# Shimly-2/DRL-on-robot-arm

Measured on AMD Instinct MI355X. Metric: env-steps/sec at N parallel envs (rl_reach_env), higher is better.
Workload: dtype f64

## Files before the change

drl-on-robot-arm_amd/csrc/armenv_env.h:

```cpp
#pragma once
#include "../../include/armenv.h"
#include "armenv_kin.h"
#include "armenv_actor.h"

using namespace armenv;


template <typename T> struct EnvCold {
  T q_init[NJ];
  T p_init[3];
  T trig_init[2 * NJ];
  T lim[2 * NJ + 1];
  double goal_lo[3], goal_hi[3];
  double push_rest_z, push_place_min, push_place_max, push_place_z;
  uint64_t seed, env_id0;
  int32_t push_model;
  int32_t fall_on;
  int32_t fall_land;
  T fall_c;
  T fall_keep;
  T place_z;
  T tool_radius, tool_below, erp_dt, split, fric_dv, dt;
};

// ... 266 lines not shown
    P.episode[i] = ep + 1u;
    if (goal_in) {
      g[0] = goal_in[3 * i]; g[1] = goal_in[3 * i + 1]; g[2] = goal_in[3 * i + 2];
    } else {
      sample_goal(P, i, ep, g);
    }
    static_for<0, NJ>([&](auto JI) { constexpr int j = JI; P.q[(int64_t)j * P.n + i] = P.cold->q_init[j]; });
    static_for<0, 2 * NJ>([&](auto JI) { constexpr int j = JI; P.trig[(int64_t)j * P.n + i] = P.cold->trig_init[j]; });
    static_for<0, 3>([&](auto KI) { constexpr int k = KI; P.goal[(int64_t)k * P.n + i] = g[k]; });
    P.step[i] = 0;
    P.ep_return[i] = T(0);
    if (obs) store_obs6<T>(obs, i, P.cold->p_init, g);
  }

  static AE_DEV double summary_distance(const EnvParams<T> &P, int64_t i) {
    T q[NJ], cq[NJ], sq[NJ];
    static_for<0, NJ>([&](auto JI) { constexpr int j = JI; q[j] = P.q[(int64_t)j * P.n + i]; });
    sincos_all<T>(q, cq, sq);
    FKState<T> S;
    fk<C, T>(P.chain, cq, sq, S);
    const T x = S.p[0] - (T)P.goal[0 * P.n + i], y = S.p[1] - (T)P.goal[1 * P.n + i], z = S.p[2] - (T)P.goal[2 * P.n + i];
    return (double)M::sqrt(M::fma(x, x, M::fma(y, y, z * z)));
  }

  T q[NJ];
  T cq[NJ], sq[NJ];
  FKState<T> S;
  AE_DEV void make_frame(const EnvParams<T> &P) { fk<C, T>(P.chain, cq, sq, S); }
  float g[3];
  int32_t step;
  T ep_ret;
  uint32_t n_done = 0, n_succ = 0, n_bad = 0, n_upd = 0;
  uint32_t n_lim = 0, n_low = 0, n_cap = 0, n_cond = 0;
  T minpiv = T(1e30);

  AE_DEV void load(const EnvParams<T> &P, int64_t i) {
    const int64_t n = P.n;
    static_for<0, NJ>([&](auto JI) { constexpr int j = JI; q[j] = P.q[(int64_t)j * n + i]; });
    static_for<0, 3>([&](auto KI) { constexpr int k = KI; g[k] = P.goal[(int64_t)k * n + i]; });
    step = P.step[i];
    ep_ret = P.ep_return[i];
    static_for<0, NJ>([&](auto JI) { constexpr int j = JI; cq[j] = P.trig[(int64_t)j * n + i]; sq[j] = P.trig[(int64_t)(NJ + j) * n + i]; });
  }
  AE_DEV void derive_trig() { sincos_all<T>(q, cq, sq); }

  AE_DEV void store(const EnvParams<T> &P, int64_t i) {
    const int64_t n = P.n;
    static_for<0, NJ>([&](auto JI) { constexpr int j = JI; P.q[(int64_t)j * n + i] = q[j]; });
    static_for<0, NJ>([&](auto JI) { constexpr int j = JI; P.trig[(int64_t)j * n + i] = cq[j]; P.trig[(int64_t)(NJ + j) * n + i] = sq[j]; });
    P.step[i] = step;
    P.ep_return[i] = ep_ret;
    flush_counts(P, i, n_done, n_succ, n_bad, n_upd, n_lim, n_low, n_cap, n_cond);
  }

  template <bool CARRY>
  AE_DEV void step_begin(const EnvParams<T> &P, const T (&a)[3], T (&tgt)[3]) {
    if constexpr (!CARRY) make_frame(P);
    ik_target<T, false>(S, a, P.dv, P.box_lo, P.box_hi, tgt);
    minpiv = T(1e30);
  }
  template <bool CARRY>
  AE_DEV void step_tail(const EnvParams<T> &P, int64_t i, const StepIO &io, int updates, bool lim_hit) {
    const int64_t n = P.n;
    n_upd += (uint32_t)updates;
    if constexpr (kFence) {
      n_lim += lim_hit ? 1u : 0u; n_low += (S.p[2] < P.fence_z) ? 1u : 0u; n_cap += (updates >= P.ik.max_iters) ? 1u : 0u;
      n_cond += (minpiv < P.ik.fence_pivot) ? 1u : 0u;
      if (io.updates) io.updates[i] = (uint8_t)(updates > 255 ? 255 : updates);
    }
    step += 1;
    const T dx = S.p[0] - (T)g[0], dy = S.p[1] - (T)g[1], dz = S.p[2] - (T)g[2];
    const T dist = M::sqrt(M::fma(dx, dx, M::fma(dy, dy, dz * dz)));
    const bool over = step > P.max_steps;
    const bool succ = !over & (dist < P.reach_dis);
    const bool done = over | succ;
    const T reward = succ ? T(0) : -dist * T(10);
    ep_ret += reward;
    if constexpr (kTipOf(kMode)) {
      if (io.diag) { io.diag[4 * i] = (double)S.p[0]; io.diag[4 * i + 1] = (double)S.p[1]; io.diag[4 * i + 2] = (double)S.p[2]; io.diag[4 * i + 3] = (double)reward; }
    }

    bool finite = true;
    {
      const T sum = ((q[0] + q[1]) + (q[2] + q[3])) + ((q[4] + q[5]) + q[6]);
      finite = M::finite(sum);
    }
    if (!finite) n_bad += 1;

    io.reward[i] = (float)reward;
    io.done[i] = done ? 1 : 0;
    io.success[i] = succ ? 1 : 0;
    if (__builtin_expect(io.terminal_obs != nullptr, 0)) store_obs6<T>(io.terminal_obs, i, S.p, g);

    const bool rederive = kTrigRederive > 0 && (step & (kTrigRederive - 1)) == 0;
    store_obs6<T>(io.obs, i, S.p, g);
    cur_obs[0] = (float)S.p[0]; cur_obs[1] = (float)S.p[1]; cur_obs[2] = (float)S.p[2];
    if (__builtin_expect(done | rederive, 0)) {
      if (done) {
        P.last_return[i] = ep_ret;
        P.last_len[i] = step;
        P.last_success[i] = succ ? 1 : 0;
        n_done += 1;
        if (succ) n_succ += 1;
      }
      if (done && P.auto_reset) {
        const uint32_t ep = P.episode[i];
        sample_goal(P, i, ep, g);
        P.episode[i] = ep + 1u;
        static_for<0, 3>([&](auto KI) { constexpr int k = KI; P.goal[(int64_t)k * n + i] = g[k]; });
        const EnvCold<T> &K = *P.cold;
        static_for<0, NJ>([&](auto JI) { constexpr int j = JI; q[j] = K.q_init[j]; });
        static_for<0, NJ>([&](auto JI) { constexpr int j = JI; cq[j] = K.trig_init[j]; sq[j] = K.trig_init[NJ + j]; });
        step = 0;
        ep_ret = T(0);
        store_obs6<T>(io.obs, i, K.p_init, g);
        cur_obs[0] = (float)K.p_init[0]; cur_obs[1] = (float)K.p_init[1]; cur_obs[2] = (float)K.p_init[2];
        if constexpr (CARRY) make_frame(P);
      } else if (rederive) {
        derive_trig();
        if constexpr (CARRY) make_frame(P);
      }
    }
  }
  template <bool CARRY = false, int PEEL = 0>
  AE_DEV int env_step(const EnvParams<T> &P, int64_t i, const T (&a)[3], const StepIO &io, ActionPrefetch *prefetched = nullptr,
                    float (*next_action)[3] = nullptr) {
    T tgt[3];
    step_begin<CARRY>(P, a, tgt);
    const int updates = ik_lockstep<C, T, kMode, PEEL>(P.chain, P.ik, q, tgt, S, cq, sq, minpiv);
    const bool lim_hit = ik_limits<C, T, kMode>(P.chain, P.ik, q, S, cq, sq);
    if (prefetched) prefetch_settle(*prefetched, *next_action);
    step_tail<CARRY>(P, i, io, updates, lim_hit);
    return updates;
  }

  float cur_obs[3];
  AE_DEV void refresh_obs(const EnvParams<T> &P) {
    FKState<T> F;
    fk<C, T>(P.chain, cq, sq, F);
    cur_obs[0] = (float)F.p[0]; cur_obs[1] = (float)F.p[1]; cur_obs[2] = (float)F.p[2];
  }
  AE_DEV void policy_obs(float (&s)[6]) const {
    s[0] = cur_obs[0]; s[1] = cur_obs[1]; s[2] = cur_obs[2]; s[3] = g[0]; s[4] = g[1]; s[5] = g[2];
  }
};

template <bool PICK, typename T>
AE_DEV void cube_sample(const EnvParams<T> &P, int64_t i, uint32_t episode, T (&cube)[3], T (&target)[3]) {
  const EnvCold<T> &K = *P.cold;
  double cx = 0, cy = 0, tx = 0, ty = 0, tz = K.push_place_z;
  constexpr uint32_t kBlocks = PICK ? 4u : 3u;
  for (uint32_t t = 0; t < 1000u; ++t) {
    double u0, u1, u2, u3, u4, u5;
    philox_pair(K.seed, K.env_id0 + (uint64_t)i, episode, kBlocks * t + 0u, u0, u1);
    philox_pair(K.seed, K.env_id0 + (uint64_t)i, episode, kBlocks * t + 1u, u2, u3);
    philox_pair(K.seed, K.env_id0 + (uint64_t)i, episode, kBlocks * t + 2u, u4, u5);
    cx = K.goal_lo[0] + (K.goal_hi[0] - K.goal_lo[0]) * u0;
    cy = K.goal_lo[1] + (K.goal_hi[1] - K.goal_lo[1]) * u1;
    tx = K.goal_lo[0] + (K.goal_hi[0] - K.goal_lo[0]) * u3;
    ty = K.goal_lo[1] + (K.goal_hi[1] - K.goal_lo[1]) * u4;
    const double dx = cx - tx, dy = cy - ty;
    double d;
    if constexpr (PICK) {
      tz = K.goal_lo[2] + (K.goal_hi[2] - K.goal_lo[2]) * u5;
      const double dz = K.push_place_z - tz;
      d = ::sqrt(::fma(dx, dx, ::fma(dy, dy, dz * dz)));
    } else {
// ... 182 lines not shown
      cube[2] = z < P.push_rest_z ? P.push_rest_z : z;
      return;
    }
    if (grip == T(0)) {
      const T h = P.push_cube_half;
      T g2 = T(0);
      static_for<0, 3>([&](auto KI) {
        constexpr int k = KI;
        const T lo = cube[k] - h, hi = cube[k] + h;
        const T c = tip[k] < lo ? lo : (tip[k] > hi ? hi : tip[k]);
        const T g = tip[k] - c;
        g2 = M::fma(g, g, g2);
      });
      if (M::sqrt(g2) - P.push_eef_radius < P.pick_trigger_dis) {
        const T hx = cube[0] - tip[0], hy = cube[1] - tip[1];
        const bool hold = tip[2] >= cube[2] && M::sqrt(M::fma(hx, hx, hy * hy)) <= P.pick_jaw_half;
        grip = hold ? T(2) : T(1);
        if (hold) {
          off[0] = hx; off[1] = hy; off[2] = cube[2] - tip[2];
          return;
        }
      }
    }
    contact(P, tip0, tip);
  }

  T p0[3];
  T q7s, c7s, s7s;
  template <bool CARRY>
  AE_DEV void step_begin(const EnvParams<T> &P, const T (&a)[3], T (&tgt)[3]) {
    if constexpr (PICK) { q7s = q[NJ - 1]; c7s = cq[NJ - 1]; s7s = sq[NJ - 1]; }
    if constexpr (!(CARRY && !PICK)) make_frame(P);
    p0[0] = S.p[0]; p0[1] = S.p[1]; p0[2] = S.p[2];
    ik_target<T, PICK>(S, a, P.dv, P.box_lo, P.box_hi, tgt);
    minpiv = T(1e30);
  }
  template <bool CARRY>
  AE_DEV void step_tail(const EnvParams<T> &P, int64_t i, const StepIO &io, int updates, bool lim_hit) {
    constexpr bool kCarry = CARRY && !PICK;
    n_upd += (uint32_t)updates;
    if constexpr (kFence) {
      n_lim += lim_hit ? 1u : 0u; n_low += (S.p[2] < P.fence_z) ? 1u : 0u; n_cap += (updates >= P.ik.max_iters) ? 1u : 0u;
      n_cond += (minpiv < P.ik.fence_pivot) ? 1u : 0u;
      if (io.updates) io.updates[i] = (uint8_t)(updates > 255 ? 255 : updates);
    }
    if constexpr (PICK) {
      q[NJ - 1] = q7s;
      cq[NJ - 1] = c7s; sq[NJ - 1] = s7s;
      const EnvCold<T> *Kp = P.cold;
      asm volatile("" : "+s"(Kp));
      if (Kp->fall_on && grip != T(2)) {
        if (step > 0) cube_fall(*Kp, 2 * step + 1);
        cube_fall(*Kp, 2 * step + 2);
      }
      grip_step(P, p0, S);
    } else {
      const EnvCold<T> *Kp = P.cold;
      asm volatile("" : "+s"(Kp));
      const EnvCold<T> &K = *Kp;
      if (K.push_model == 1) { cube_fall(K, step + 2); contact_dyn(P, K, S.p, step + 2); }
      else contact(P, p0, S.p);
    }
    step += 1;
    const T d_cur = dist_ct();
    T test = d_cur - d_last;
    if (M::fabs(test) < T(1e-5)) test = T(0.01);
    d_last = d_cur;
    const float fx = (float)cube[0] - (float)target[0], fy = (float)cube[1] - (float)target[1],
                fz = (float)cube[2] - (float)target[2];
    const float dt32 = sqrtf(fmaf(fx, fx, fmaf(fy, fy, fz * fz)));
    T reward;
    bool done;
    if (step > P.max_steps) { reward = (T)(-dt32 * 50.0f); done = true; }
    else if ((double)dt32 < (double)P.push_success_dis) { reward = T(100); done = true; }
    else { reward = -test * T(100); done = false; }
    const bool succ = d_cur < P.push_success_dis;
    ep_ret += reward;
    if constexpr (kTipOf(kMode)) {
      if (io.diag) { io.diag[4 * i] = (double)S.p[0]; io.diag[4 * i + 1] = (double)S.p[1]; io.diag[4 * i + 2] = (double)S.p[2]; io.diag[4 * i + 3] = (double)reward; }
    }

    bool finite = true;
    {
      const T sum = ((q[0] + q[1]) + (q[2] + q[3])) + ((q[4] + q[5]) + q[6]);
      finite = M::finite(sum);
    }
    if (!finite) n_bad += 1;

    io.reward[i] = (float)reward;
    io.done[i] = done ? 1 : 0;
    io.success[i] = succ ? 1 : 0;
    if (__builtin_expect(io.terminal_obs != nullptr, 0)) store_obs9<T>(io.terminal_obs, i, S.p, cube, target);
    const bool rederive = kTrigRederive > 0 && (step & (kTrigRederive - 1)) == 0;
    store_obs9<T>(io.obs, i, S.p, cube, target);
    cur_obs[0] = (float)S.p[0]; cur_obs[1] = (float)S.p[1]; cur_obs[2] = (float)S.p[2];
    if (__builtin_expect(done | rederive, 0)) {
      if (done) {
        P.last_return[i] = ep_ret;
        P.last_len[i] = step;
        P.last_success[i] = succ ? 1 : 0;
        n_done += 1;
        if (succ) n_succ += 1;
      }
      if (done && P.auto_reset) {
        const uint32_t ep = P.episode[i];
        cube_sample<PICK, T>(P, i, ep, cube, target);
        P.episode[i] = ep + 1u;
        d_last = dist_ct();
        if constexpr (PICK) { grip = T(0); off[0] = off[1] = off[2] = T(0); }
        else { vel[0] = vel[1] = T(0); }
        const EnvCold<T> &K = *P.cold;
        static_for<0, NJ>([&](auto JI) { constexpr int j = JI; q[j] = K.q_init[j]; });
        static_for<0, NJ>([&](auto JI) { constexpr int j = JI; cq[j] = K.trig_init[j]; sq[j] = K.trig_init[NJ + j]; });
        step = 0;
        ep_ret = T(0);
        store_obs9<T>(io.obs, i, K.p_init, cube, target);
        cur_obs[0] = (float)K.p_init[0]; cur_obs[1] = (float)K.p_init[1]; cur_obs[2] = (float)K.p_init[2];
        if constexpr (kCarry) make_frame(P);
      } else if (rederive) {
        derive_trig();
        if constexpr (kCarry) make_frame(P);
      }
    }
  }
  template <bool CARRY = false, int PEEL = 0>
  AE_DEV int env_step(const EnvParams<T> &P, int64_t i, const T (&a)[3], const StepIO &io, ActionPrefetch *prefetched = nullptr,
                    float (*next_action)[3] = nullptr) {
    T tgt[3];
    step_begin<CARRY>(P, a, tgt);
    const int updates = ik_lockstep<C, T, kMode, PEEL>(P.chain, P.ik, q, tgt, S, cq, sq, minpiv);
    const bool lim_hit = ik_limits<C, T, kMode>(P.chain, P.ik, q, S, cq, sq);
    if (prefetched) prefetch_settle(*prefetched, *next_action);
    step_tail<CARRY>(P, i, io, updates, lim_hit);
    return updates;
  }
};
template <class C, typename T, int MODE = 0> using PushLane = CubeLane<C, T, false, MODE>;
template <class C, typename T, int MODE = 0> using PickLane = CubeLane<C, T, true, MODE>;

template <class Lane, typename T>
__global__ __launch_bounds__(256) void env_reset_kernel(EnvParams<T> P, const uint8_t *mask, const float *goal_in, float *obs) {
  const int64_t i = (int64_t)blockIdx.x * blockDim.x + threadIdx.x;
  if (i >= P.n) return;
  if (mask && !mask[i]) return;
  Lane::reset_env(P, i, goal_in, obs);
}

template <class Lane, typename T, int WAVES = 1>
__global__ __launch_bounds__(256) __attribute__((amdgpu_waves_per_eu(WAVES, WAVES))) void env_step_kernel(EnvParams<T> P, StepIO io) {
  TL_STAMP(tl0);
#ifdef ARMENV_TIMELINE
  const unsigned tl_launch = __hip_atomic_load(&g_tl_launch, __ATOMIC_RELAXED, __HIP_MEMORY_SCOPE_AGENT);
#endif
  const int64_t i = lane_env(P);
  if (i < 0) return;
  if (i >= P.n) return;
  Lane L;
  L.load(P, i);
  T a[3];
  static_for<0, 3>([&](auto KI) { constexpr int k = KI; a[k] = (T)io.action[3 * i + k]; });
#ifdef ARMENV_TIMELINE
  asm volatile("s_waitcnt vmcnt(0)" ::: "memory");
#endif
  TL_STAMP(tl1);
  const int updates = L.template env_step<false, ARMENV_STEP_PEEL>(P, i, a, io);
  (void)updates;
  TL_STAMP(tl2);
// ... 343 lines not shown
```

drl-on-robot-arm_amd/csrc/armenv_kin.h:

```cpp
#pragma once
#include "armenv_math.h"
#include "chains_builtin.h"

namespace armenv {

constexpr bool kFenceOf(int mode) { return mode >= 1; }
constexpr bool kTipOf(int mode) { return mode == 2; }

template <typename T> struct ChainDev {
  T xyz[NJ][3];
  T R[NJ][9];
  T base_p[3];
  T base_R[9];
};

struct GenericChain {
  static constexpr bool kGeneric = true;
  static constexpr const char *kName = "generic";
};

template <typename T> struct IKParams {
  T tq[4];
  T lambda;
  T residual;
  T max_dtheta;
  int32_t max_iters;
  int32_t exit_mode;
  int32_t angle_f32;
  int32_t clamp_limits;
  int32_t pad0;
  T fence_pivot;
  T tip[3];
  const T *lim;
  T lim_min;
};

template <typename T> struct FKState {
  T W[9];
  T p[3];
  T z[NJ][3];
  T pj[NJ][3];
};

template <class C> struct FkKinds {
  int Wk[NJ + 1][9];
  int Ak[NJ][9];
  constexpr FkKinds() : Wk{}, Ak{} {
    for (int i = 0; i < 9; ++i) Wk[0][i] = (i % 4 == 0) ? 2 : 1;
    for (int j = 0; j < NJ; ++j) {
      for (int c = 0; c < 3; ++c) {
        const int k = C::perm[j][c], sg = C::sgn[j][c];
        for (int r = 0; r < 3; ++r) {
          const int w = Wk[j][3 * k + r];
          Ak[j][3 * c + r] = (sg > 0 || w < 2) ? w : (w == 2 ? 3 : 2);
        }
      }
      for (int r = 0; r < 3; ++r) {
        const bool z = Ak[j][r] == 1 && Ak[j][3 + r] == 1;
        Wk[j + 1][r] = z ? 1 : 0;
        Wk[j + 1][3 + r] = z ? 1 : 0;
        Wk[j + 1][6 + r] = Ak[j][6 + r];
      }
    }
  }
};
template <int KA, int KB, typename T>
AE_DEV T rot_term(T c, T a, T s, T b) {
  using M = Mth<T>;
  if constexpr (KA == 1 && KB == 1) return T(0);
  else if constexpr (KA == 1) return KB == 2 ? s : (KB == 3 ? -s : s * b);
  else if constexpr (KB == 1) return KA == 2 ? c : (KA == 3 ? -c : c * a);
  else if constexpr (KA >= 2) return (KA == 2 ? c : -c) + (KB == 2 ? s : (KB == 3 ? -s : s * b));
  else return M::fma(c, a, KB == 2 ? s : (KB == 3 ? -s : s * b));
}

template <class C, typename T>
AE_DEV void fk(const ChainDev<T> &ch, const T (&cq)[NJ], const T (&sq)[NJ], FKState<T> &S) {
  using M = Mth<T>;
  if constexpr (C::kGeneric) {
    static_for<0, 9>([&](auto I) { constexpr int i = I; S.W[3 * (i % 3) + (i / 3)] = ch.base_R[i]; });
    static_for<0, 3>([&](auto I) { constexpr int i = I; S.p[i] = ch.base_p[i]; });
  } else {
    static_for<0, 9>([&](auto I) { constexpr int i = I; S.W[i] = (i % 4 == 0) ? T(1) : T(0); });
    static_for<0, 3>([&](auto I) { constexpr int i = I; S.p[i] = T(0); });
  }
  static_for<0, NJ>([&](auto JI) {
    constexpr int j = JI;
    T A[9];
    if constexpr (C::kGeneric) {
      static_for<0, 3>([&](auto RI) {
        constexpr int r = RI;
        S.p[r] = M::fma(S.W[0 + r], ch.xyz[j][0], M::fma(S.W[3 + r], ch.xyz[j][1], M::fma(S.W[6 + r], ch.xyz[j][2], S.p[r])));
      });
      static_for<0, 3>([&](auto CI) {
        constexpr int c = CI;
        static_for<0, 3>([&](auto RI) {
          constexpr int r = RI;
          A[3 * c + r] = M::fma(S.W[0 + r], ch.R[j][0 + c], M::fma(S.W[3 + r], ch.R[j][3 + c], S.W[6 + r] * ch.R[j][6 + c]));
        });
      });
    } else {
      static_for<0, 3>([&](auto KI) {
        constexpr int k = KI;
        constexpr double t = C::xyz[j][k];
        if constexpr (t != 0.0) {
          static_for<0, 3>([&](auto RI) {
            constexpr int r = RI;
            constexpr int kw = FkKinds<C>().Wk[j][3 * k + r];
            if constexpr (kw == 0) S.p[r] = M::fma(S.W[3 * k + r], T(t), S.p[r]);
            else if constexpr (kw == 2) S.p[r] = S.p[r] + T(t);
            else if constexpr (kw == 3) S.p[r] = S.p[r] - T(t);
          });
        }
      });
      static_for<0, 3>([&](auto CI) {
        constexpr int c = CI;
        constexpr int k = C::perm[j][c];
        constexpr int s = C::sgn[j][c];
        static_for<0, 3>([&](auto RI) { constexpr int r = RI; A[3 * c + r] = (s > 0) ? S.W[3 * k + r] : -S.W[3 * k + r]; });
      });
    }
    const T sn = sq[j], cs = cq[j];
    static_for<0, 3>([&](auto RI) {
      constexpr int r = RI;
      if constexpr (C::kGeneric) {
        S.W[0 + r] = M::fma(cs, A[0 + r], sn * A[3 + r]);
        S.W[3 + r] = M::fma(cs, A[3 + r], -(sn * A[0 + r]));
      } else {
        constexpr int k0 = FkKinds<C>().Ak[j][0 + r], k3 = FkKinds<C>().Ak[j][3 + r];
        constexpr int k0n = k0 < 2 ? k0 : (k0 == 2 ? 3 : 2);
        S.W[0 + r] = rot_term<k0, k3, T>(cs, A[0 + r], sn, A[3 + r]);
        S.W[3 + r] = rot_term<k3, k0n, T>(cs, A[3 + r], sn, -A[0 + r]);
      }
      S.W[6 + r] = A[6 + r];
      S.z[j][r] = A[6 + r];
      S.pj[j][r] = S.p[r];
    });
  });
}

template <typename T>
AE_DEV void sincos_kernel(T r, T &s, T &c) {
  using M = Mth<T>;
  const T z = r * r;
  T ps = T(1.58969099521155010221e-10);
  ps = M::fma(ps, z, T(-2.50507602534068634195e-08));
  ps = M::fma(ps, z, T(2.75573137070700676789e-06));
  ps = M::fma(ps, z, T(-1.98412698298579493134e-04));
  ps = M::fma(ps, z, T(8.33333333332248946124e-03));
  ps = M::fma(ps, z, T(-1.66666666666666324348e-01));
  s = M::fma(r * z, ps, r);
  T pc = T(-1.13596475577881948265e-11);
  pc = M::fma(pc, z, T(2.08757232129817482790e-09));
  pc = M::fma(pc, z, T(-2.75573143513906633035e-07));
  pc = M::fma(pc, z, T(2.48015872894767294178e-05));
  pc = M::fma(pc, z, T(-1.38888888888741095749e-03));
  pc = M::fma(pc, z, T(4.16666666666666019037e-02));
  c = M::fma(z * z, pc, M::fma(T(-0.5), z, T(1)));
}

AE_DEV void sincos_joint(double x, double &s, double &c) {
  if (!(::fabs(x) < 1.0e5)) { ::sincos(x, &s, &c); return; }
  const double k = ::rint(x * 6.36619772367581382433e-01);
  double r = ::fma(-k, 1.57079632673412561417e+00, x);
  r = ::fma(-k, 6.07710050630396597660e-11, r);
  r = ::fma(-k, 2.02226624871116645580e-21, r);
  r = ::fma(-k, 8.47842766036889956997e-32, r);
  double sr, cr;
  sincos_kernel<double>(r, sr, cr);
  const int n = (int)k & 3;
  const double s1 = (n & 1) ? cr : sr, c1 = (n & 1) ? sr : cr;
  s = (n & 2) ? -s1 : s1;
  c = ((n + 1) & 2) ? -c1 : c1;
}
AE_DEV void sincos_joint(float x, float &s, float &c) { ::sincosf(x, &s, &c); }

template <typename T>
AE_DEV void sincos_all(const T (&q)[NJ], T (&cq)[NJ], T (&sq)[NJ]) {
  static_for<0, NJ>([&](auto JI) { constexpr int j = JI; sincos_joint(q[j], sq[j], cq[j]); });
}
template <>
AE_DEV void sincos_all<double>(const double (&q)[NJ], double (&cq)[NJ], double (&sq)[NJ]) {
  double k[NJ], r[NJ], z[NJ], ps[NJ], pc[NJ];
  static_for<0, NJ>([&](auto JI) { constexpr int j = JI; k[j] = ::rint(q[j] * 6.36619772367581382433e-01); });
  static_for<0, NJ>([&](auto JI) { constexpr int j = JI; r[j] = ::fma(-k[j], 1.57079632673412561417e+00, q[j]); });
  static_for<0, NJ>([&](auto JI) { constexpr int j = JI; r[j] = ::fma(-k[j], 6.07710050630396597660e-11, r[j]); });
  static_for<0, NJ>([&](auto JI) { constexpr int j = JI; r[j] = ::fma(-k[j], 2.02226624871116645580e-21, r[j]); });
  static_for<0, NJ>([&](auto JI) { constexpr int j = JI; r[j] = ::fma(-k[j], 8.47842766036889956997e-32, r[j]); z[j] = r[j] * r[j]; });
  static_for<0, NJ>([&](auto JI) { constexpr int j = JI; ps[j] = ::fma(1.58969099521155010221e-10, z[j], -2.50507602534068634195e-08); });
  static_for<0, NJ>([&](auto JI) { constexpr int j = JI; ps[j] = ::fma(ps[j], z[j], 2.75573137070700676789e-06); });
  static_for<0, NJ>([&](auto JI) { constexpr int j = JI; ps[j] = ::fma(ps[j], z[j], -1.98412698298579493134e-04); });
  static_for<0, NJ>([&](auto JI) { constexpr int j = JI; ps[j] = ::fma(ps[j], z[j], 8.33333333332248946124e-03); });
  static_for<0, NJ>([&](auto JI) { constexpr int j = JI; ps[j] = ::fma(ps[j], z[j], -1.66666666666666324348e-01); });
  static_for<0, NJ>([&](auto JI) { constexpr int j = JI; pc[j] = ::fma(-1.13596475577881948265e-11, z[j], 2.08757232129817482790e-09); });
  static_for<0, NJ>([&](auto JI) { constexpr int j = JI; pc[j] = ::fma(pc[j], z[j], -2.75573143513906633035e-07); });
  static_for<0, NJ>([&](auto JI) { constexpr int j = JI; pc[j] = ::fma(pc[j], z[j], 2.48015872894767294178e-05); });
  static_for<0, NJ>([&](auto JI) { constexpr int j = JI; pc[j] = ::fma(pc[j], z[j], -1.38888888888741095749e-03); });
  static_for<0, NJ>([&](auto JI) { constexpr int j = JI; pc[j] = ::fma(pc[j], z[j], 4.16666666666666019037e-02); });
  static_for<0, NJ>([&](auto JI) {
    constexpr int j = JI;
    const double sr = ::fma(r[j] * z[j], ps[j], r[j]);
    const double cr = ::fma(z[j] * z[j], pc[j], ::fma(-0.5, z[j], 1.0));
    const int n = (int)k[j] & 3;
    const double s1 = (n & 1) ? cr : sr, c1 = (n & 1) ? sr : cr;
    sq[j] = (n & 2) ? -s1 : s1;
    cq[j] = ((n + 1) & 2) ? -c1 : c1;
  });
}
template <>
AE_DEV void sincos_all<float>(const float (&q)[NJ], float (&cq)[NJ], float (&sq)[NJ]) {
  float k[NJ], r[NJ], z[NJ], ps[NJ], pc[NJ];
  static_for<0, NJ>([&](auto JI) { constexpr int j = JI; k[j] = ::rintf(q[j] * 0.636619772f); });
  static_for<0, NJ>([&](auto JI) { constexpr int j = JI; r[j] = ::fmaf(-k[j], 1.5703125f, q[j]); });
  static_for<0, NJ>([&](auto JI) { constexpr int j = JI; r[j] = ::fmaf(-k[j], 4.837512969970703125e-4f, r[j]); });
  static_for<0, NJ>([&](auto JI) { constexpr int j = JI; r[j] = ::fmaf(-k[j], 7.54978995489188216e-8f, r[j]); z[j] = r[j] * r[j]; });
  static_for<0, NJ>([&](auto JI) { constexpr int j = JI; ps[j] = ::fmaf(2.7183114939898219064e-6f, z[j], -1.98393348360966317347e-4f); });
  static_for<0, NJ>([&](auto JI) { constexpr int j = JI; ps[j] = ::fmaf(ps[j], z[j], 8.3333293858894631756e-3f); });
  static_for<0, NJ>([&](auto JI) { constexpr int j = JI; ps[j] = ::fmaf(ps[j], z[j], -1.66666666416265235595e-1f); });
  static_for<0, NJ>([&](auto JI) { constexpr int j = JI; pc[j] = ::fmaf(2.43904487962774090654e-5f, z[j], -1.38867637746099294692e-3f); });
  static_for<0, NJ>([&](auto JI) { constexpr int j = JI; pc[j] = ::fmaf(pc[j], z[j], 4.16666233237390631894e-2f); });
  static_for<0, NJ>([&](auto JI) { constexpr int j = JI; pc[j] = ::fmaf(pc[j], z[j], -4.99999997251031003120e-1f); });
  static_for<0, NJ>([&](auto JI) {
    constexpr int j = JI;
    const float sr = ::fmaf(r[j] * z[j], ps[j], r[j]);
    const float cr = ::fmaf(z[j], pc[j], 1.0f);
    const int n = (int)k[j] & 3;
    const float s1 = (n & 1) ? cr : sr, c1 = (n & 1) ? sr : cr;
    sq[j] = (n & 2) ? -s1 : s1;
    cq[j] = ((n + 1) & 2) ? -c1 : c1;
  });
}

template <typename T>
AE_DEV void rotate_small(T &c, T &s, T d) {
  using M = Mth<T>;
  T sd, cd;
  sincos_kernel<T>(d, sd, cd);
  const T cn = M::fma(c, cd, -(s * sd));
  const T sn = M::fma(s, cd, c * sd);
  c = cn;
  s = sn;
}

AE_DEV double hw_rcp(double x) { return __builtin_amdgcn_rcp(x); }
AE_DEV float hw_rcp(float x) { return __builtin_amdgcn_rcpf(x); }
AE_DEV double hw_rsq(double x) { return __builtin_amdgcn_rsq(x); }
AE_DEV float hw_rsq(float x) { return __builtin_amdgcn_rsqf(x); }

template <typename T>
AE_DEV T fast_rcp(T d) {
#ifdef ARMENV_EXACT_RCP
  return T(1) / d;
#endif
  T r = hw_rcp(d);
  r = Mth<T>::fma(Mth<T>::fma(-d, r, T(1)), r, r);
  if constexpr (sizeof(T) == 8) r = Mth<T>::fma(Mth<T>::fma(-d, r, T(1)), r, r);
  return r;
}

template <typename T>
AE_DEV T fast_rsqrt(T x) {
#ifdef ARMENV_EXACT_RSQRT
  return T(1) / Mth<T>::sqrt(x);
#endif
  T r = hw_rsq(x);
  const T hx = T(0.5) * x;
  r = Mth<T>::fma(Mth<T>::fma(-hx * r, r, T(0.5)), r, r);
  if constexpr (sizeof(T) == 8) r = Mth<T>::fma(Mth<T>::fma(-hx * r, r, T(0.5)), r, r);
  return r;
}

template <typename T>
AE_DEV void quat_from_frame(const T (&W)[9], T (&q)[4]) {
  const T m00 = W[0], m10 = W[1], m20 = W[2], m01 = W[3], m11 = W[4], m21 = W[5], m02 = W[6], m12 = W[7], m22 = W[8];
  const T trace = m00 + m11 + m22;
  const bool cw = trace > T(0);
  const bool cz = !cw & (m00 < m11 ? (m11 < m22) : (m00 < m22));
  const bool cy = !cw & !cz & (m00 < m11);
  const T tw = trace + T(1), tz = m22 - m00 - m11 + T(1), ty = m11 - m22 - m00 + T(1), tx = m00 - m11 - m22 + T(1);
  const T t = cw ? tw : (cz ? tz : (cy ? ty : tx));
  const T h = T(0.5) * fast_rsqrt<T>(t);
  const T big = t * h;
  const T d21 = (m21 - m12) * h, d02 = (m02 - m20) * h, d10 = (m10 - m01) * h;
  T s10 = (m10 + m01) * h, s20 = (m20 + m02) * h, s21 = (m21 + m12) * h;
  asm("" : "+v"(s10), "+v"(s20), "+v"(s21));
  q[0] = cw ? d21 : (cz ? s20 : (cy ? s10 : big));
  q[1] = cw ? d02 : (cz ? s21 : (cy ? big : s10));
  q[2] = cw ? d10 : (cz ? big : (cy ? s21 : s20));
  q[3] = cw ? big : (cz ? d10 : (cy ? d02 : d21));
}

AE_DEV double acos_branchfree(double x) {
#ifdef ARMENV_EXACT_ACOS
  return ::acos(x);
#endif
  const double ax = ::fabs(x);
  const bool small = ax < 0.5;
  const double z = small ? x * x : ::fma(-0.5, ax, 0.5);
  double p = ::fma(3.47933107596021167570e-05, z, 7.91534994289814532176e-04);
  p = ::fma(p, z, -4.00555345006794114027e-02);
  p = ::fma(p, z, 2.01212532134862925881e-01);
  p = ::fma(p, z, -3.25565818622400915405e-01);
  p = ::fma(p, z, 1.66666666666666657415e-01);
  p = p * z;
  double q = ::fma(7.70381505559019352791e-02, z, -6.88283971605453293030e-01);
  q = ::fma(q, z, 2.02094576023350569471e+00);
  q = ::fma(q, z, -2.40339491173441421878e+00);
  q = ::fma(q, z, 1.0);
  const double R = p * fast_rcp<double>(q);
  const double sr = z * fast_rsqrt<double>(small ? 1.0 : (z > 0.0 ? z : 1.0));
  const double s = z > 0.0 ? sr : 0.0;
  const double pio2_hi = 1.57079632679489655800e+00, pio2_lo = 6.12323399573676603587e-17;
  const double inner = pio2_hi - (x - ::fma(-x, R, pio2_lo));
  const double w = ::fma(R, s, s);
  const double outer = x < 0.0 ? ::fma(-2.0, w - pio2_lo, 3.14159265358979311600e+00) : 2.0 * w;
  return small ? inner : outer;
}

template <typename T>
AE_DEV void orientation_error(const T (&tq)[4], const T (&qc)[4], int angle_f32, T (&e)[3]) {
  using M = Mth<T>;
  const T bx = -qc[0], by = -qc[1], bz = -qc[2], bw = qc[3];
  const T ax = tq[0], ay = tq[1], az = tq[2], aw = tq[3];
  const T dx = M::fma(aw, bx, M::fma(ax, bw, M::fma(ay, bz, -(az * by))));
  const T dy = M::fma(aw, by, M::fma(ay, bw, M::fma(az, bx, -(ax * bz))));
  const T dz = M::fma(aw, bz, M::fma(az, bw, M::fma(ax, by, -(ay * bx))));
  const T dw = M::fma(aw, bw, -M::fma(ax, bx, M::fma(ay, by, az * bz)));
  if constexpr (sizeof(T) == 4) {
    const T sg = dw < T(0) ? T(-1) : T(1);
    const T n = M::sqrt(M::fma(dx, dx, M::fma(dy, dy, dz * dz)));
    const T ang = T(2) * ::atan2f(n, sg * dw);
    const T k = n > T(1e-30) ? sg * ang / n : T(0);
    e[0] = k * dx; e[1] = k * dy; e[2] = k * dz;
    return;
  }
  const T wc = dw < T(-1) ? T(-1) : (dw > T(1) ? T(1) : dw);
  T angle = T(2) * (T)acos_branchfree((double)wc);
  const T s2 = M::fma(-dw, dw, T(1));
  const T v2 = M::fma(dx, dx, M::fma(dy, dy, dz * dz));
  const bool degenerate = (s2 < T(10) * M::eps) || !(v2 > T(0));
  const T rv = fast_rsqrt<T>(degenerate ? T(1) : v2);
  if (angle_f32) angle = (T)(float)angle;
  angle = angle > M::pi ? angle - T(2) * M::pi : angle;
  if (angle_f32) angle = (T)(float)angle;
  e[0] = degenerate ? angle : angle * (dx * rv);
  e[1] = degenerate ? T(0) : angle * (dy * rv);
  e[2] = degenerate ? T(0) : angle * (dz * rv);
}

template <class C, bool G = C::kGeneric> struct Axis0 { static constexpr int m = 2, sg = 1; };
template <class C> struct Axis0<C, false> { static constexpr int m = C::perm[0][2], sg = C::sgn[0][2]; };
template <class C> constexpr int k0_kind(int row) {
  if (C::kGeneric) return 0;
  const int m = Axis0<C>::m, sg = Axis0<C>::sg;
  if (row < 3) return row == m ? 1 : 0;
  return (row - 3 == m) ? (sg > 0 ? 2 : 3) : 1;
}
template <class C, bool G = C::kGeneric> struct ZKind { static constexpr int of(int, int) { return 0; } };
template <class C> struct ZKind<C, false> { static constexpr int of(int k, int r) { return FkKinds<C>().Ak[k][6 + r]; } };
template <class C> constexpr int col_kind(int k, int row) {
  if (k == 0) return k0_kind<C>(row);
  return row < 3 ? 0 : ZKind<C>::of(k, row - 3);
}
template <class C, typename T, int K, int R, int CC>
AE_DEV T jj_term(T a, T b, T acc) {
  constexpr int ka = col_kind<C>(K, R), kb = col_kind<C>(K, CC);
  if constexpr (ka == 1 || kb == 1) return acc;
  else if constexpr (ka >= 2 && kb >= 2) return acc + ((ka == kb) ? T(1) : T(-1));
  else if constexpr (ka == 2) return acc + b;
  else if constexpr (ka == 3) return acc - b;
  else if constexpr (kb == 2) return acc + a;
  else if constexpr (kb == 3) return acc - a;
  else return Mth<T>::fma(a, b, acc);
}
template <class C, typename T, int MODE = 0>
AE_DEV void dls_update(const FKState<T> &S, const T (&pe)[3], const T (&e)[6], const IKParams<T> &P, T (&dth)[NJ], T &minpiv) {
  using M = Mth<T>;
  constexpr bool FENCE = kFenceOf(MODE);
  constexpr int NL = kTipOf(MODE) ? NJ : NJ - 1;
  T Jl[NL][3];
  static_for<0, NL>([&](auto II) {
    constexpr int i = II;
    const T r0 = pe[0] - S.pj[i][0], r1 = pe[1] - S.pj[i][1], r2 = pe[2] - S.pj[i][2];
    if constexpr (i == 0 && !C::kGeneric) {
      constexpr int m = Axis0<C>::m, sg = Axis0<C>::sg;
      const T r[3] = {r0, r1, r2};
      Jl[0][m] = T(0);
      Jl[0][(m + 1) % 3] = sg > 0 ? -r[(m + 2) % 3] : r[(m + 2) % 3];
      Jl[0][(m + 2) % 3] = sg > 0 ? r[(m + 1) % 3] : -r[(m + 1) % 3];
    } else {
      constexpr int kz0 = ZKind<C>::of(i, 0), kz1 = ZKind<C>::of(i, 1), kz2 = ZKind<C>::of(i, 2);
      constexpr auto neg = [](int k) constexpr { return k < 2 ? k : (k == 2 ? 3 : 2); };
      Jl[i][0] = rot_term<kz1, neg(kz2), T>(r2, S.z[i][1], r1, -S.z[i][2]);
      Jl[i][1] = rot_term<kz2, neg(kz0), T>(r0, S.z[i][2], r2, -S.z[i][0]);
      Jl[i][2] = rot_term<kz0, neg(kz1), T>(r1, S.z[i][0], r0, -S.z[i][1]);
    }
  });
  T A[6][6];
  static_for<0, 6>([&](auto RI) {
    constexpr int r = RI;
    static_for<0, r + 1>([&](auto CI) {
      constexpr int c = CI;
      T acc = (r == c) ? P.lambda : T(0);
      static_for<0, (r < 3 || c < 3) ? NL : NJ>([&](auto KI) {
        constexpr int k = KI;
        const T a = (r < 3) ? Jl[k < NL ? k : 0][r % 3] : S.z[k][r % 3];
        const T b = (c < 3) ? Jl[k < NL ? k : 0][c % 3] : S.z[k][c % 3];
        acc = jj_term<C, T, k, r, c>(a, b, acc);
      });
      A[r][c] = acc;
    });
  });
  T L[6][6], invD[6], D[6];
  static_for<0, 6>([&](auto JI) {
    constexpr int j = JI;
    T v[6];
    T d = A[j][j];
    static_for<0, j>([&](auto KI) {
      constexpr int k = KI;
      v[k] = L[j][k] * D[k];
      d = M::fma(-L[j][k], v[k], d);
    });
    D[j] = d;
    invD[j] = fast_rcp<T>(d);
    static_for<j + 1, 6>([&](auto II) {
      constexpr int i = II;
      T s = A[i][j];
      static_for<0, j>([&](auto KI) {
        constexpr int k = KI;
        s = M::fma(-L[i][k], v[k], s);
      });
      L[i][j] = s * invD[j];
    });
  });
  if constexpr (FENCE) {
    const T m = M::fmin(M::fmin(M::fmin(D[0], D[1]), M::fmin(D[2], D[3])), M::fmin(D[4], D[5]));
    minpiv = M::fmin(minpiv, m);
  }
  T y[6];
  static_for<0, 6>([&](auto II) {
    constexpr int i = II;
    T s = e[i];
    static_for<0, i>([&](auto KI) { constexpr int k = KI; s = M::fma(-L[i][k], y[k], s); });
    y[i] = s;
  });
  static_for<0, 6>([&](auto II) { constexpr int i = II; y[i] *= invD[i]; });
  static_for<0, 6>([&](auto II) {
    constexpr int i = 5 - II;
    T s = y[i];
    static_for<i + 1, 6>([&](auto KI) { constexpr int k = KI; s = M::fma(-L[k][i], y[k], s); });
    y[i] = s;
  });
  T mx = T(0);
  static_for<0, NJ>([&](auto II) {
    constexpr int i = II;
    T s;
    if constexpr (i == 0 && !C::kGeneric) {
      s = T(0);
      bool first = true;
      static_for<0, 6>([&](auto RI) {
        constexpr int r = RI;
        constexpr int kind = k0_kind<C>(r);
        const T a = (r < 3) ? Jl[0][r % 3] : S.z[0][r % 3];
        if constexpr (kind == 0) { s = first ? a * y[r] : M::fma(a, y[r], s); first = false; }
        else if constexpr (kind == 2) { s = first ? y[r] : s + y[r]; first = false; }
        else if constexpr (kind == 3) { s = first ? -y[r] : s - y[r]; first = false; }
      });
    } else if constexpr (i < NL) {
      s = Jl[i][0] * y[0];
      s = M::fma(Jl[i][1], y[1], s);
      s = M::fma(Jl[i][2], y[2], s);
      static_for<0, 3>([&](auto RI) {
        constexpr int r = RI;
        constexpr int kz = ZKind<C>::of(i, r);
        if constexpr (kz == 0) s = M::fma(S.z[i][r], y[3 + r], s);
        else if constexpr (kz == 2) s = s + y[3 + r];
        else if constexpr (kz == 3) s = s - y[3 + r];
      });
    } else {
      s = S.z[i][0] * y[3];
      s = M::fma(S.z[i][1], y[4], s);
      s = M::fma(S.z[i][2], y[5], s);
    }
    dth[i] = s;
    mx = M::fmax(mx, M::fabs(s));
  });
  const bool over = mx > P.max_dtheta;
  const T sc = over ? P.max_dtheta * fast_rcp<T>(over ? mx : T(1)) : T(1);
  static_for<0, NJ>([&](auto II) { constexpr int i = II; dth[i] = dth[i] * sc; });
}

template <typename T, bool START_F32>
AE_DEV void ik_target(const FKState<T> &S, const T (&a)[3], T dv, const T (&box_lo)[3], const T (&box_hi)[3], T (&tgt)[3]) {
  using M = Mth<T>;
  static_for<0, 3>([&](auto KI) {
    constexpr int k = KI;
    T v = M::fma(a[k], dv, START_F32 ? (T)(float)S.p[k] : S.p[k]);
    v = v < box_lo[k] ? box_lo[k] : v;
    v = v > box_hi[k] ? box_hi[k] : v;
    tgt[k] = v;
  });
}
template <class C, typename T, int MODE = 0>
AE_DEV bool ik_stop(const IKParams<T> &P, const T (&tgt)[3], const FKState<T> &S, T diff2_prev, int it, T res2, T (&e)[6], T (&pe)[3],
                    T &diff2) {
  using M = Mth<T>;
  static_for<0, 3>([&](auto RI) {
    constexpr int r = RI;
    if constexpr (kTipOf(MODE)) pe[r] = M::fma(S.W[0 + r], P.tip[0], M::fma(S.W[3 + r], P.tip[1], M::fma(S.W[6 + r], P.tip[2], S.p[r])));
    else pe[r] = S.p[r];
  });
  e[0] = tgt[0] - pe[0];
  e[1] = tgt[1] - pe[1];
  e[2] = tgt[2] - pe[2];
  diff2 = M::fma(e[0], e[0], M::fma(e[1], e[1], e[2] * e[2]));
  int em = P.exit_mode;
  asm("" : "+v"(em));
  const T dtest = em == 0 ? diff2_prev : diff2;
  return (it >= P.max_iters) | !(dtest > res2);
}
template <class C, typename T, int MODE = 0, int SMALL = -1>
AE_DEV void ik_update(const ChainDev<T> &ch, const IKParams<T> &P, T (&q)[NJ], FKState<T> &S, T (&cq)[NJ], T (&sq)[NJ], T (&e)[6],
                      const T (&pe)[3], T diff2, T &diff2_prev, int &it, bool small_steps, T &minpiv) {
  T qc[4], eo[3], dth[NJ];
  quat_from_frame<T>(S.W, qc);
  orientation_error<T>(P.tq, qc, P.angle_f32, eo);
  e[3] = eo[0]; e[4] = eo[1]; e[5] = eo[2];
  dls_update<C, T, MODE>(S, pe, e, P, dth, minpiv);
  static_for<0, NJ>([&](auto II) { constexpr int i = II; q[i] += dth[i]; });
  if constexpr (SMALL >= 0) small_steps = SMALL != 0;
#ifdef ARMENV_EXACT_ROTATE
  small_steps = false;
#endif
  if (__builtin_expect(small_steps, 1)) {
    static_for<0, NJ>([&](auto II) { constexpr int i = II; rotate_small<T>(cq[i], sq[i], dth[i]); });
  } else {
    sincos_all<T>(q, cq, sq);
  }
  diff2_prev = diff2;
  ++it;
  fk<C, T>(ch, cq, sq, S);
}
template <class C, typename T, int MODE = 0, int SMALL = -1>
AE_DEV bool ik_trip(const ChainDev<T> &ch, const IKParams<T> &P, T (&q)[NJ], const T (&tgt)[3], FKState<T> &S, T (&cq)[NJ],
                    T (&sq)[NJ], T &diff2_prev, int &it, T res2, bool small_steps, T &minpiv) {
  T e[6], pe[3], diff2;
  if (ik_stop<C, T, MODE>(P, tgt, S, diff2_prev, it, res2, e, pe, diff2)) return true;
  ik_update<C, T, MODE, SMALL>(ch, P, q, S, cq, sq, e, pe, diff2, diff2_prev, it, small_steps, minpiv);
  return false;
}
template <class C, typename T, int MODE = 0, int PEEL = 0>
AE_DEV int ik_lockstep(const ChainDev<T> &ch, const IKParams<T> &P, T (&q)[NJ], const T (&tgt)[3], FKState<T> &S, T (&cq)[NJ],
                       T (&sq)[NJ], T &minpiv) {
  const T res2 = P.residual * P.residual;
  const bool small_steps = P.max_dtheta <= T(0.7854);
  T diff2_prev = T(1e60);
  int it = 0;
  bool stopped = false;
  static_for<0, PEEL>([&](auto) {
    if (!stopped) stopped = ik_trip<C, T, MODE>(ch, P, q, tgt, S, cq, sq, diff2_prev, it, res2, small_steps, minpiv);
  });
  if (!stopped) while (!ik_trip<C, T, MODE>(ch, P, q, tgt, S, cq, sq, diff2_prev, it, res2, small_steps, minpiv)) {}
  return it;
}

template <class C, typename T, int MODE = 0>
AE_DEV bool ik_limits(const ChainDev<T> &ch, const IKParams<T> &P, T (&q)[NJ], FKState<T> &S, T (&cq)[NJ], T (&sq)[NJ]) {
  using M = Mth<T>;
  constexpr bool FENCE = kFenceOf(MODE);
  bool hit = false;
  if (FENCE || __builtin_expect(P.clamp_limits != 0, 0)) {
// ... 50 lines not shown
```

Measured before the change: 11.43 billion.

## Trim selects in quaternion, rsqrt guards, and z-axis storage in FK/IK

Several micro-optimizations land together. FK now stores the joint z axis from the pre-rotation W column and leaves the sign flip to the Jacobian, and the quaternion extraction uses two booleans with sign-selected sums instead of nested selects. Guard selects around rsqrt/rcp inputs are dropped, and an asm barrier is added on the finiteness sum. Each aims to shave VALU instructions or register pressure per step, but dropping the guards can let degenerate inputs produce inf or NaN that the later selects must mask.

After: 11.52 billion (median of 5 runs). No clear change (+0.7%).

```diff
diff --git a/drl-on-robot-arm_amd/csrc/armenv_env.h b/drl-on-robot-arm_amd/csrc/armenv_env.h
--- a/drl-on-robot-arm_amd/csrc/armenv_env.h
+++ b/drl-on-robot-arm_amd/csrc/armenv_env.h
@@ -372,7 +372,8 @@
 
     bool finite = true;
     {
-      const T sum = ((q[0] + q[1]) + (q[2] + q[3])) + ((q[4] + q[5]) + q[6]);
+      T sum = ((q[0] + q[1]) + (q[2] + q[3])) + ((q[4] + q[5]) + q[6]);
+      asm volatile("" : "+v"(sum));
       finite = M::finite(sum);
     }
     if (!finite) n_bad += 1;
@@ -721,7 +722,8 @@
 
     bool finite = true;
     {
-      const T sum = ((q[0] + q[1]) + (q[2] + q[3])) + ((q[4] + q[5]) + q[6]);
+      T sum = ((q[0] + q[1]) + (q[2] + q[3])) + ((q[4] + q[5]) + q[6]);
+      asm volatile("" : "+v"(sum));
       finite = M::finite(sum);
     }
     if (!finite) n_bad += 1;
diff --git a/drl-on-robot-arm_amd/csrc/armenv_kin.h b/drl-on-robot-arm_amd/csrc/armenv_kin.h
--- a/drl-on-robot-arm_amd/csrc/armenv_kin.h
+++ b/drl-on-robot-arm_amd/csrc/armenv_kin.h
@@ -41,6 +41,8 @@
   T z[NJ][3];
   T pj[NJ][3];
 };
+template <class C, bool G = C::kGeneric> struct ZSgn { static constexpr int of(int) { return 1; } };
+template <class C> struct ZSgn<C, false> { static constexpr int of(int j) { return C::sgn[j][2]; } };
 
 template <class C> struct FkKinds {
   int Wk[NJ + 1][9];
@@ -119,6 +121,7 @@
         constexpr int s = C::sgn[j][c];
         static_for<0, 3>([&](auto RI) { constexpr int r = RI; A[3 * c + r] = (s > 0) ? S.W[3 * k + r] : -S.W[3 * k + r]; });
       });
+      static_for<0, 3>([&](auto RI) { constexpr int r = RI; S.z[j][r] = S.W[3 * C::perm[j][2] + r]; });
     }
     const T sn = sq[j], cs = cq[j];
     static_for<0, 3>([&](auto RI) {
@@ -133,7 +136,7 @@
         S.W[3 + r] = rot_term<k3, k0n, T>(cs, A[3 + r], sn, -A[0 + r]);
       }
       S.W[6 + r] = A[6 + r];
-      S.z[j][r] = A[6 + r];
+      if constexpr (C::kGeneric) S.z[j][r] = A[6 + r];
       S.pj[j][r] = S.p[r];
     });
   });
@@ -280,14 +283,18 @@
   const T tw = trace + T(1), tz = m22 - m00 - m11 + T(1), ty = m11 - m22 - m00 + T(1), tx = m00 - m11 - m22 + T(1);
   const T t = cw ? tw : (cz ? tz : (cy ? ty : tx));
   const T h = T(0.5) * fast_rsqrt<T>(t);
-  const T big = t * h;
-  const T d21 = (m21 - m12) * h, d02 = (m02 - m20) * h, d10 = (m10 - m01) * h;
-  T s10 = (m10 + m01) * h, s20 = (m20 + m02) * h, s21 = (m21 + m12) * h;
-  asm("" : "+v"(s10), "+v"(s20), "+v"(s21));
-  q[0] = cw ? d21 : (cz ? s20 : (cy ? s10 : big));
-  q[1] = cw ? d02 : (cz ? s21 : (cy ? big : s10));
-  q[2] = cw ? d10 : (cz ? big : (cy ? s21 : s20));
-  q[3] = cw ? big : (cz ? d10 : (cy ? d02 : d21));
+  const bool b0 = !cw & (cz | !(m00 < m11));
+  const bool b1 = !cw & !cz;
+  T x0 = (m21 + ((b0 != b1) ? m12 : -m12)) * h;
+  T x1 = (m02 + (b0 ? m20 : -m20)) * h;
+  T x2 = (m10 + (b1 ? m01 : -m01)) * h;
+  T x3 = t * h;
+  asm("" : "+v"(x0), "+v"(x1), "+v"(x2), "+v"(x3));
+  const T y0 = b0 ? x1 : x0, y1 = b0 ? x0 : x1, y2 = b0 ? x3 : x2, y3 = b0 ? x2 : x3;
+  q[0] = b1 ? y2 : y0;
+  q[1] = b1 ? y3 : y1;
+  q[2] = b1 ? y0 : y2;
+  q[3] = b1 ? y1 : y3;
 }
 
 AE_DEV double acos_branchfree(double x) {
@@ -308,7 +315,7 @@
   q = ::fma(q, z, -2.40339491173441421878e+00);
   q = ::fma(q, z, 1.0);
   const double R = p * fast_rcp<double>(q);
-  const double sr = z * fast_rsqrt<double>(small ? 1.0 : (z > 0.0 ? z : 1.0));
+  const double sr = z * fast_rsqrt<double>(z);
   const double s = z > 0.0 ? sr : 0.0;
   const double pio2_hi = 1.57079632679489655800e+00, pio2_lo = 6.12323399573676603587e-17;
   const double inner = pio2_hi - (x - ::fma(-x, R, pio2_lo));
@@ -339,7 +346,7 @@
   const T s2 = M::fma(-dw, dw, T(1));
   const T v2 = M::fma(dx, dx, M::fma(dy, dy, dz * dz));
   const bool degenerate = (s2 < T(10) * M::eps) || !(v2 > T(0));
-  const T rv = fast_rsqrt<T>(degenerate ? T(1) : v2);
+  const T rv = fast_rsqrt<T>(v2);
   if (angle_f32) angle = (T)(float)angle;
   angle = angle > M::pi ? angle - T(2) * M::pi : angle;
   if (angle_f32) angle = (T)(float)angle;
@@ -378,6 +385,11 @@
   using M = Mth<T>;
   constexpr bool FENCE = kFenceOf(MODE);
   constexpr int NL = kTipOf(MODE) ? NJ : NJ - 1;
+  T z[NJ][3];
+  static_for<0, NJ>([&](auto II) {
+    constexpr int i = II;
+    static_for<0, 3>([&](auto RI) { constexpr int r = RI; z[i][r] = ZSgn<C>::of(i) < 0 ? -S.z[i][r] : S.z[i][r]; });
+  });
   T Jl[NL][3];
   static_for<0, NL>([&](auto II) {
     constexpr int i = II;
@@ -391,9 +403,9 @@
     } else {
       constexpr int kz0 = ZKind<C>::of(i, 0), kz1 = ZKind<C>::of(i, 1), kz2 = ZKind<C>::of(i, 2);
       constexpr auto neg = [](int k) constexpr { return k < 2 ? k : (k == 2 ? 3 : 2); };
-      Jl[i][0] = rot_term<kz1, neg(kz2), T>(r2, S.z[i][1], r1, -S.z[i][2]);
-      Jl[i][1] = rot_term<kz2, neg(kz0), T>(r0, S.z[i][2], r2, -S.z[i][0]);
-      Jl[i][2] = rot_term<kz0, neg(kz1), T>(r1, S.z[i][0], r0, -S.z[i][1]);
+      Jl[i][0] = rot_term<kz1, neg(kz2), T>(r2, z[i][1], r1, -z[i][2]);
+      Jl[i][1] = rot_term<kz2, neg(kz0), T>(r0, z[i][2], r2, -z[i][0]);
+      Jl[i][2] = rot_term<kz0, neg(kz1), T>(r1, z[i][0], r0, -z[i][1]);
     }
   });
   T A[6][6];
@@ -404,8 +416,8 @@
       T acc = (r == c) ? P.lambda : T(0);
       static_for<0, (r < 3 || c < 3) ? NL : NJ>([&](auto KI) {
         constexpr int k = KI;
-        const T a = (r < 3) ? Jl[k < NL ? k : 0][r % 3] : S.z[k][r % 3];
-        const T b = (c < 3) ? Jl[k < NL ? k : 0][c % 3] : S.z[k][c % 3];
+        const T a = (r < 3) ? Jl[k < NL ? k : 0][r % 3] : z[k][r % 3];
+        const T b = (c < 3) ? Jl[k < NL ? k : 0][c % 3] : z[k][c % 3];
         acc = jj_term<C, T, k, r, c>(a, b, acc);
       });
       A[r][c] = acc;
@@ -461,7 +473,7 @@
       static_for<0, 6>([&](auto RI) {
         constexpr int r = RI;
         constexpr int kind = k0_kind<C>(r);
-        const T a = (r < 3) ? Jl[0][r % 3] : S.z[0][r % 3];
+        const T a = (r < 3) ? Jl[0][r % 3] : z[0][r % 3];
         if constexpr (kind == 0) { s = first ? a * y[r] : M::fma(a, y[r], s); first = false; }
         else if constexpr (kind == 2) { s = first ? y[r] : s + y[r]; first = false; }
         else if constexpr (kind == 3) { s = first ? -y[r] : s - y[r]; first = false; }
@@ -473,20 +485,20 @@
       static_for<0, 3>([&](auto RI) {
         constexpr int r = RI;
         constexpr int kz = ZKind<C>::of(i, r);
-        if constexpr (kz == 0) s = M::fma(S.z[i][r], y[3 + r], s);
+        if constexpr (kz == 0) s = M::fma(z[i][r], y[3 + r], s);
         else if constexpr (kz == 2) s = s + y[3 + r];
         else if constexpr (kz == 3) s = s - y[3 + r];
       });
     } else {
-      s = S.z[i][0] * y[3];
-      s = M::fma(S.z[i][1], y[4], s);
-      s = M::fma(S.z[i][2], y[5], s);
+      s = z[i][0] * y[3];
+      s = M::fma(z[i][1], y[4], s);
+      s = M::fma(z[i][2], y[5], s);
     }
     dth[i] = s;
     mx = M::fmax(mx, M::fabs(s));
   });
   const bool over = mx > P.max_dtheta;
-  const T sc = over ? P.max_dtheta * fast_rcp<T>(over ? mx : T(1)) : T(1);
+  const T sc = over ? P.max_dtheta * fast_rcp<T>(mx) : T(1);
   static_for<0, NJ>([&](auto II) { constexpr int i = II; dth[i] = dth[i] * sc; });
 }
 
```
